# hsinnan75/GSAlign

Hardware: AMD Instinct MI355X
Metric: aligned query Gbp/s (whole node) (higher is better)
Workload: dtype u8; 1 GPU; full-human-sized pair (BASELINE configs[4]): 24 contigs with GRCh38 chromosome lengths, 3.08 Gbp, repeat injection, vs 1; inflight_contexts_per_gpu=8, world_size=1, parallelism=one GPU

## Files before the change

### gsalign_amd/csrc/k_seed.hip

```cpp
#include <cstring>
#include <mutex>
#include <condition_variable>
#include <vector>
#include "gsa_ctx.h"
#include "gsa_fm.h"
#include "gsa_scan.h"

enum { CNT_OCCBLK = 0, CNT_DONE = 1, CNT_HITS = 2, CNT_SEEDS = 3, CNT_DPCELLS = 4, CNT_DPJOBS = 5, CNT_DPMN = 6, CNT_CAND = 8, CNT_OVERFLOW = 9, CNT_OCCBLK_ALL = 10, CNT_HEAVY = 12 };

#ifndef SEED_WG
#define SEED_WG 64
#endif
#ifndef NSUB
#define NSUB 96
#endif
#ifndef ADV_STEPS
#define ADV_STEPS 4
#endif
#ifndef PLOOK
#define PLOOK 3
#endif
#define PATH_WORDS 320
#define QP_WORDS (GSA_CHUNK / 16 + 4)
#define QN_WORDS (GSA_CHUNK / 32 + 4)
// ... 8 lines not shown
{
	const u64 lo = (u64)w0 | ((u64)w1 << 32);
	return sh ? (lo >> sh) | ((u64)w2 << (64 - sh)) : lo;
}
__device__ __forceinline__ u64 q_bits64(const u32 *qp, int p) { const int w = p >> 4; return funnel64(qp[w], qp[w + 1], qp[w + 2], (p & 15) << 1); }
__device__ __forceinline__ u32 q_nbits32(const u32 *qn, int p) { const int w = p >> 5; return (u32)((((u64)qn[w + 1] << 32) | qn[w]) >> (p & 31)); }

__device__ __forceinline__ int text_match32(u32 r0, u32 r1, u32 r2, i64 tp, i64 tend, const u32 *qp, const u32 *qn, int pos, int clen)
{
	int avail = clen - pos;
	if (tend - tp < (i64)avail) avail = (int)(tend - tp);
	if (avail > 32) avail = 32;
	if (avail <= 0) return 0;
	const u64 d = funnel64(r0, r1, r2, (int)(tp & 15) << 1) ^ q_bits64(qp, pos);
	const u64 dm = (d | (d >> 1)) & 0x5555555555555555ull;
	const u32 nm = q_nbits32(qn, pos);
	int n = dm ? (__ffsll((unsigned long long)dm) - 1) >> 1 : 32;
	const int fn = nm ? __ffs((int)nm) - 1 : 32;
	n = n < fn ? n : fn;
	return n < avail ? n : avail;
}

__device__ __forceinline__ u32 pres4_line(u64 qb, int K) { return (u32)((qb >> 6) & ((1ull << (2 * (K - 3))) - 1)); }
__device__ __forceinline__ u32 pres4_bit(u64 qb, int K, int i)
{
	const u32 head = (u32)(qb >> (2 * i)) & ((1u << (2 * (3 - i))) - 1);
	const u32 tail = (u32)(qb >> (2 * K)) & ((1u << (2 * i)) - 1);
	return (u32)i * 64u + (head | (tail << (2 * (3 - i))));
}

template <int TPB>
__device__ __forceinline__ void wg_exscan_hits(const i32 *hits, i32 *base, int n1)
{
	constexpr int V = TPB <= 64 ? 16 : 8;
	__shared__ i32 s_ws[TPB / 64], s_run;
	const int tid = threadIdx.x, lane = tid & 63, wv = tid >> 6;
	if (tid == 0) s_run = 0;
	__syncthreads();
	for (int b0 = 0; b0 < n1; b0 += TPB * V) {
		i32 v[V], tsum = 0;
#pragma unroll
		for (int k = 0; k < V; k++) { const int idx = b0 + tid * V + k; v[k] = idx < n1 ? __hip_atomic_load(&hits[idx], __ATOMIC_RELAXED, __HIP_MEMORY_SCOPE_AGENT) : 0; }
#pragma unroll
		for (int k = 0; k < V; k++) tsum += v[k];
		i32 inc = tsum;
		for (int o = 1; o < 64; o <<= 1) { const i32 t = __shfl_up(inc, o); if (lane >= o) inc += t; }
		if (lane == 63) s_ws[wv] = inc;
		__syncthreads();
		i32 wo = 0, tot = 0;
		for (int w = 0; w < TPB / 64; w++) { const i32 x = s_ws[w]; if (w < wv) wo += x; tot += x; }
		i32 e = s_run + wo + inc - tsum;
#pragma unroll
		for (int k = 0; k < V; k++) { const int idx = b0 + tid * V + k; if (idx < n1) base[idx] = e; e += v[k]; }
		__syncthreads();
		if (tid == 0) s_run += tot;
		__syncthreads();
	}
}

__device__ __forceinline__ void wave_exscan_hits(const i32 *hits, i32 *base, int n1)
{
	constexpr int V = 16;
	const int lane = threadIdx.x & 63;
	i32 run = 0;
	for (int b0 = 0; b0 < n1; b0 += 64 * V) {
		i32 v[V], tsum = 0;
#pragma unroll
		for (int k = 0; k < V; k++) { const int idx = b0 + lane * V + k; v[k] = idx < n1 ? __hip_atomic_load(&hits[idx], __ATOMIC_RELAXED, __HIP_MEMORY_SCOPE_AGENT) : 0; }
#pragma unroll
		for (int k = 0; k < V; k++) tsum += v[k];
		i32 inc = tsum;
		for (int o = 1; o < 64; o <<= 1) { const i32 t = __shfl_up(inc, o); if (lane >= o) inc += t; }
		i32 e = run + inc - tsum;
#pragma unroll
		for (int k = 0; k < V; k++) { const int idx = b0 + lane * V + k; if (idx < n1) base[idx] = e; e += v[k]; }
		run += __shfl(inc, 63);
	}
}

#ifndef SEED_MIN_WAVES
#define SEED_MIN_WAVES 5
#endif
#ifndef LHOP_N
#define LHOP_N 1024
#endif
#define MEMO_WORDS (GSA_CHUNK / 16)
__device__ __forceinline__ int memo_nib(const u32 *memo, int s) { return (int)((memo[s >> 4] >> ((s & 15) << 1)) & 3u); }
__device__ __forceinline__ void memo_one(u32 *memo, int s) { atomicOr(&memo[s >> 4], 1u << ((s & 15) << 1)); }
__device__ __forceinline__ int memo_get(const u32 *memo, const u32 *lhop, int s)
{
	const int v = memo_nib(memo, s);
	if (v < 2) return v;
	if (v == 2) return 5;
	for (u32 h = ((u32)s * 40503u) >> 6;; h++) { const u32 e = lhop[h & (LHOP_N - 1)]; if ((e >> 16) == (u32)s + 1) return (int)(e & 0xffffu); }
}
__device__ __forceinline__ void memo_set(u32 *memo, u32 *lhop, int s, int d, int *abort_flag)
{
	if (d == 1 || d == 5) { atomicOr(&memo[s >> 4], (d == 1 ? 1u : 2u) << ((s & 15) << 1)); return; }
	const u32 e = ((u32)(s + 1) << 16) | (u32)d;
	u32 h = ((u32)s * 40503u) >> 6;
	for (int tries = 0; tries < LHOP_N; tries++, h++) {
		const u32 old = atomicCAS(&lhop[h & (LHOP_N - 1)], 0u, e);
		if (old == 0 || old == e) { atomicOr(&memo[s >> 4], 3u << ((s & 15) << 1)); return; }
	}
	*(volatile int *)abort_flag = 1;
}

__device__ __forceinline__ u32 nt4_quad(u32 w)
{
	const u32 l = w | 0x20202020u;
	const u32 x = (l >> 1) & 0x03030303u;
	u32 code = x ^ ((x >> 1) & 0x01010101u);
	const u32 want = __builtin_amdgcn_perm(0u, 0x74676361u, code);
	const u32 diff = l ^ want;
	const u32 bad = ((diff | ((diff & 0x7f7f7f7fu) + 0x7f7f7f7fu)) >> 7) & 0x01010101u;
	code &= ~(bad * 3u);
	return ((code * 0x01041040u) >> 24) | (((bad * 0x01020408u) >> 24) & 15u) << 8;
}

__device__ __forceinline__ void stage32(const uint8_t *src, int p0, int clen, u32 &w0, u32 &w1, u32 &wn)
{
	u32 d[8];
	if (p0 + 32 <= clen) { const uint4 a = *(const uint4 *)src, b = *(const uint4 *)(src + 16); d[0] = a.x; d[1] = a.y; d[2] = a.z; d[3] = a.w; d[4] = b.x; d[5] = b.y; d[6] = b.z; d[7] = b.w; }
	else {
#pragma unroll
		for (int t = 0; t < 8; t++) { d[t] = 0; for (int k = 0; k < 4; k++) d[t] |= (u32)(p0 + 4 * t + k < clen ? src[4 * t + k] : (uint8_t)'N') << (8 * k); }
	}
	w0 = w1 = wn = 0;
#pragma unroll
	for (int t = 0; t < 8; t++) {
		const u32 r = nt4_quad(d[t]);
		if (t < 4) w0 |= (r & 0xffu) << (8 * t); else w1 |= (r & 0xffu) << (8 * (t - 4));
		wn |= (r >> 8) << (4 * t);
	}
}

template <bool COUNT, int NCH>
struct SeedLds {
	static constexpr int NV = NCH * NSUB;
	u32 s_ncand[NCH], s_queue, s_hits[NCH];
	int changed, s_abort;
	u32 qp[NCH][QP_WORDS], qn[NCH][QN_WORDS];
	u32 memo[NCH][MEMO_WORDS];
	u32 lhop[NCH][LHOP_N];
	uint16_t mblk[COUNT ? GSA_CHUNK : 1];
	u32 bits[NCH][PATH_WORDS];
	uint16_t entry_of[NV], exit_of[NV];
	uint16_t pend_it[SEED_WG];
	uint16_t jmp[2][NV], walked_from[NV];
	u32 rewalked[(NV + 31) / 32], onchain[(NV + 31) / 32], s_npend;
	int s_last;
};
#define SEED_SYNC() do { if (WPW == 1) __syncthreads(); else { __builtin_amdgcn_fence(__ATOMIC_RELEASE, "wavefront"); __builtin_amdgcn_wave_barrier(); __builtin_amdgcn_fence(__ATOMIC_ACQUIRE, "wavefront"); } } while (0)
#define s_ncand sl_.s_ncand
#define s_queue sl_.s_queue
#define s_hits sl_.s_hits
#define changed sl_.changed
#define s_abort sl_.s_abort
#define qp sl_.qp
#define qn sl_.qn
#define memo sl_.memo
#define lhop sl_.lhop
#define mblk sl_.mblk
#define bits sl_.bits
#define entry_of sl_.entry_of
#define exit_of sl_.exit_of
#define pend_it sl_.pend_it
#define jmp sl_.jmp
#define walked_from sl_.walked_from
#define rewalked sl_.rewalked
#define onchain sl_.onchain
#define s_npend sl_.s_npend
#define s_last sl_.s_last
template <bool COUNT, bool E16, int NCH, int WPW>
__device__ __forceinline__ void seed_chunk(const DevIndex &di, const uint8_t *__restrict__ q, i32 qlen, const Params &prm, u64 *cnt,
                                                      i32 *cand_s, i32 *cand_len, u64 *cand_x0, i32 *cand_freq, u32 cand_cap, u32 *cand_cnt, u32 *onpath, i32 *chunk_hits, u64 *hcnt,
                                                      u32 budget, u32 *heavy_list, i32 *chunk_base, const int chunk0, const u32 n_chunks, SeedLds<COUNT, NCH> &sl_)
{
	constexpr int NV = NCH * NSUB;
	static_assert(!COUNT || NCH == 1, "the accounting build walks one chunk per wave");
	const int j = threadIdx.x & 63;
	const int nch = (u32)chunk0 + NCH <= n_chunks ? NCH : (int)(n_chunks - (u32)chunk0);
	i64 c0[NCH]; int clen[NCH], S[NCH], nitems[NCH]; size_t cbase[NCH];
#pragma unroll
	for (int ch = 0; ch < NCH; ch++) {
		c0[ch] = (i64)(chunk0 + ch) * GSA_CHUNK;
		clen[ch] = ch < nch ? (int)((i64)qlen - c0[ch] < GSA_CHUNK ? (i64)qlen - c0[ch] : GSA_CHUNK) : 0;
		S[ch] = (clen[ch] + NSUB - 1) / NSUB; if (S[ch] < 1) S[ch] = 1;
		nitems[ch] = (clen[ch] + S[ch] - 1) / S[ch];
		cbase[ch] = (size_t)(chunk0 + ch) * cand_cap;
	}
	const int nitems_all = NCH == 1 ? nitems[0] : nitems[0] + nitems[NCH - 1];
#define CH_SEL(ARR, CH) (NCH == 1 ? ARR[0] : ((CH) ? ARR[NCH - 1] : ARR[0]))
#pragma unroll
	for (int ch = 0; ch < NCH; ch++) {
		for (int g = j; g < QN_WORDS; g += SEED_WG) {
			u32 w0 = 0, w1 = 0, wn = 0;
			const int p0 = g << 5;
			if (p0 < clen[ch]) stage32(q + c0[ch] + p0, p0, clen[ch], w0, w1, wn);
			if (2 * g < QP_WORDS) qp[ch][2 * g] = w0;
			if (2 * g + 1 < QP_WORDS) qp[ch][2 * g + 1] = w1;
			qn[ch][g] = wn;
		}
		for (int p = j; p < MEMO_WORDS; p += SEED_WG) memo[ch][p] = 0;
		for (int p = j; p < LHOP_N; p += SEED_WG) lhop[ch][p] = 0;
		for (int p = j; p < PATH_WORDS; p += SEED_WG) bits[ch][p] = 0;
		for (int it = j; it < nitems[ch]; it += SEED_WG) entry_of[ch * NSUB + it] = (uint16_t)(it * S[ch]);
		if (j == 0) { s_ncand[ch] = 0; s_hits[ch] = 0; }
	}
	if (j == 0) { s_queue = 0; s_npend = 0; s_abort = 0; }
	if (j < (NV + 31) / 32) rewalked[j] = 0;
	u32 all_blocks = 0, rounds = 0, iters = 0;
#ifdef SEED_STATS
	u32 st_it = 0, st_fm_any = 0, st_fm_only = 0, st_act = 0, st_fm = 0;
#endif
	unsigned long long t_begin = wall_clock64(), t_round0 = 0, t_resolve = 0;
	u32 dirty = 0;
	int fb_item = 0;
	SEED_SYNC();
	for (;;) {
		int item = -1, s = 0, bend = 0, pos = 0, mode = M_ADV; u32 kid = 0, pid = 0, pext = 0;
		int lclen = 0;
		const u32 *qp_l = qp[0], *qn_l = qn[0]; u32 *memo_l = memo[0], *lhop_l = lhop[0];
		FmIntv ik = {0, 0, 0}; u32 blk = 0; i64 tp = 0;
		i64 mp[4] = {0, 0, 0, 0}; u32 malive = 0;
		bool need_item = true;
		while (!__all(mode == M_DONE)) {
			iters++;
			if (!COUNT && budget && iters > budget) *(volatile int *)&s_abort = 1;
			if (*(volatile int *)&s_abort) break;
#ifdef SEED_STATS
			{ const u64 bf = __ballot(mode == M_FM), ba = __ballot(mode != M_DONE);
			  st_it++; st_fm_any += bf != 0; st_fm_only += bf != 0 && bf == ba; st_act += __popcll(ba); st_fm += __popcll(bf); }
#endif
			u64 kk = 0, ll = 0; bool kn = true, ln = true;
			if (mode == M_FM) {
				const u64 k = ik.x1 - 1, l = ik.x1 - 1 + ik.x2;
				kn = (k == (u64)-1); ln = (l == (u64)-1);
				kk = kn ? 0 : k - (k >= di.primary); ll = ln ? 0 : l - (l >= di.primary);
			}
#ifdef SEED_SKIP_IDLE
#define ANY_IN(M) __any(mode == (M))
#else
#define ANY_IN(M) true
#endif
			FmBlock bk = {{0, 0, 0, 0}, {0, 0, 0, 0}, 0, 0, 0, 0}, bl = bk;
			if (ANY_IN(M_FM)) { bk = fm_load(di, kk >> 6); bl = fm_load(di, ll >> 6); }
			struct __attribute__((packed, aligned(4))) W5 { u32 a, b, c, d, e; };
			W5 w5 = {0, 0, 0, 0, 0};
			if (ANY_IN(M_TEXT)) w5 = *(const W5 *)(di.ref2 + (mode == M_TEXT ? (tp >> 4) : ((mode == M_MTEXT && (malive & 1u)) ? (mp[0] >> 4) : 0)));
			const u32 r0 = w5.a, r1 = w5.b, r2 = w5.c, r3 = w5.d, r4 = w5.e;
			ulonglong2 e0 = {0, 0}, e1 = {0, 0};
			if (!ANY_IN(M_KMER)) {}
			else if (E16) {
				const uint4 e = ((const uint4 *)(di.kmer ? di.kmer : (const u64 *)di.bwt))[mode == M_KMER ? kid : 0];
				e0.x = e.x; e0.y = e.y; e1.x = e.z; e1.y = e.w;
			} else {
				const ulonglong2 *pe = (const ulonglong2 *)((di.kmer ? di.kmer : (const u64 *)di.bwt) + (mode == M_KMER ? ((size_t)kid << 2) : 0));
				e0 = pe[0]; e1 = pe[1];
			}
			uint4 pl0 = {~0u, ~0u, ~0u, ~0u}, pl1 = {~0u, ~0u, ~0u, ~0u};
			if (di.pres && ANY_IN(M_KMER)) { const uint4 *pp = (const uint4 *)di.pres + 2 * (size_t)(mode == M_KMER ? pid : 0); pl0 = pp[0]; pl1 = pp[1]; }
#define PRES4_TEST(I) ((((((pext >> (2 * (I))) & 32u) ? ((I) == 0 ? pl0.y : (I) == 1 ? pl0.w : (I) == 2 ? pl1.y : pl1.w) : ((I) == 0 ? pl0.x : (I) == 1 ? pl0.z : (I) == 2 ? pl1.x : pl1.z)) >> ((pext >> (2 * (I))) & 31u)) & 1u) != 0)
			u64 sav = 0;
			if (ANY_IN(M_LOC)) sav = fm_locate(di, (mode == M_LOC || mode == M_MLOC) ? ik.x0 : 1);
#undef ANY_IN
			u64 sav1 = 0, sav2 = 0, sav3 = 0; W5 w5b = {0, 0, 0, 0, 0}, w5c = w5b, w5d = w5b;
			if (!COUNT && SEED_MULTI > 1) {
				if (__any(mode == M_MLOC)) {
					const int nr = mode == M_MLOC ? (int)ik.x2 : 0;
					sav1 = fm_locate(di, nr > 1 ? ik.x0 + 1 : 1); sav2 = fm_locate(di, nr > 2 ? ik.x0 + 2 : 1); sav3 = fm_locate(di, nr > 3 ? ik.x0 + 3 : 1);
				}
				if (__any(mode == M_MTEXT)) {
					const bool mt = mode == M_MTEXT;
					w5b = *(const W5 *)(di.ref2 + ((mt && (malive & 2u)) ? (mp[1] >> 4) : 0));
					w5c = *(const W5 *)(di.ref2 + ((mt && (malive & 4u)) ? (mp[2] >> 4) : 0));
					w5d = *(const W5 *)(di.ref2 + ((mt && (malive & 8u)) ? (mp[3] >> 4) : 0));
				}
			}
			bool ended = false;
			if (mode == M_KMER) {
				if (!PRES4_TEST(0)) {
					memo_one(memo_l, s); s += 1; mode = M_ADV;
					const int L = prm.MinSeedLength < 32 ? prm.MinSeedLength : 32;
#pragma unroll
					for (int k2 = 0; k2 < PLOOK; k2++) {
						if (s >= bend || memo_nib(memo_l, s)) break;
						const u32 nb = q_nbits32(qn_l, s);
						if (s + prm.MinSeedLength > lclen || (nb & (L == 32 ? ~0u : (1u << L) - 1)) != 0) break;
						if (k2 == 0 ? PRES4_TEST(1) : k2 == 1 ? PRES4_TEST(2) : PRES4_TEST(3)) break;
						memo_one(memo_l, s); s += 1;
					}
				} else {
					const bool hit = e1.x != 0;
					if (hit) { ik.x0 = e0.x; ik.x1 = e0.y; ik.x2 = e1.x; pos = s + di.kmer_k; }
					else ik = fm_init(di, q_code(qp_l, s));
					mode = M_FM;
					if (hit && ik.x2 == 1) { tp = (i64)(e1.y - 1) + di.kmer_k; mode = M_TEXT; }
					else if (!COUNT && SEED_MULTI > 1 && hit && ik.x2 <= SEED_MULTI) mode = M_MLOC;
				}
			} else if (mode == M_LOC) {
				tp = (i64)sav + (pos - s); mode = M_TEXT;
			} else if (!COUNT && SEED_MULTI > 1 && mode == M_MLOC) {
				mp[0] = (i64)sav + (pos - s); mp[1] = (i64)sav1 + (pos - s); mp[2] = (i64)sav2 + (pos - s); mp[3] = (i64)sav3 + (pos - s);
				malive = (1u << (int)ik.x2) - 1u; mode = M_MTEXT;
			} else if (!COUNT && SEED_MULTI > 1 && mode == M_MTEXT) {
				int g0 = -1, g1 = -1, g2 = -1, g3 = -1;
#define MT_ROW(G, W, P) { int got = text_match32(W.a, W.b, W.c, P, (i64)di.seq_len, qp_l, qn_l, pos, lclen); if (got == 32) got += text_match32(W.c, W.d, W.e, P + 32, (i64)di.seq_len, qp_l, qn_l, pos + 32, lclen); G = got; }
				if (malive & 1u) MT_ROW(g0, w5, mp[0])
				if (malive & 2u) MT_ROW(g1, w5b, mp[1])
				if (malive & 4u) MT_ROW(g2, w5c, mp[2])
				if (malive & 8u) MT_ROW(g3, w5d, mp[3])
#undef MT_ROW
				int m = g0 > g1 ? g0 : g1; m = m > g2 ? m : g2; m = m > g3 ? m : g3;
				const u32 na = (g0 == m ? 1u : 0u) | (g1 == m ? 2u : 0u) | (g2 == m ? 4u : 0u) | (g3 == m ? 8u : 0u);
				pos += m; mp[0] += m; mp[1] += m; mp[2] += m; mp[3] += m;
				if (m < 64 || __popc(na) == 1) {
					const int first = __ffs((int)na) - 1;
					ik.x0 += (u64)first; ik.x2 = (u64)__popc(na);
					if (m == 64) { tp = first == 0 ? mp[0] : first == 1 ? mp[1] : first == 2 ? mp[2] : mp[3]; mode = M_TEXT; }
					else ended = true;
				} else malive = na;
				if (mode == M_MTEXT && !ended && malive != na) malive = na;
			} else if (mode == M_TEXT) {
				int got = text_match32(r0, r1, r2, tp, (i64)di.seq_len, qp_l, qn_l, pos, lclen);
				if (got == 32) got += text_match32(r2, r3, r4, tp + 32, (i64)di.seq_len, qp_l, qn_l, pos + 32, lclen);
				pos += got; tp += got;
				ended = got < 64;
			} else if (mode == M_FM) {
				const bool can = pos < lclen && !q_isn(qn_l, pos < lclen ? pos : 0);
				const bool ok = can && fm_extend_loaded(di, ik, q_code(qp_l, pos < lclen ? pos : 0), bk, bl, kk, ll, kn, ln, blk);
				ended = !ok;
				if (ok) { pos++; if (!COUNT && ik.x2 == 1) mode = M_LOC; else if (!COUNT && SEED_MULTI > 1 && ik.x2 <= SEED_MULTI) mode = M_MLOC; }
			}
			if (ended) {
				const int len = pos - s;
				int d = 1;
				if (len >= prm.MinSeedLength && ik.x2 <= GSA_MAX_SEED_FREQ) {
					const int ch = NCH == 1 ? 0 : (item >= NSUB ? NCH - 1 : 0);
					const u32 slot = atomicAdd(&s_ncand[ch], 1u);
					const size_t cb = CH_SEL(cbase, ch);
					if (slot < cand_cap) { cand_s[cb + slot] = (i32)(CH_SEL(c0, ch) + s); cand_len[cb + slot] = len; cand_x0[cb + slot] = ik.x0; cand_freq[cb + slot] = (i32)ik.x2; }
					else cnt[CNT_OVERFLOW] = 1;
					d = prm.bSensitive ? 5 : len + 1;
				}
				memo_set(memo_l, lhop_l, s, d, &s_abort); if (COUNT) mblk[s] = (uint16_t)blk;
				all_blocks += blk;
				s += d; mode = M_ADV;
			}
			for (int step = 0; step < ADV_STEPS && mode == M_ADV; step++) {
				if (need_item) {
					if (rounds == 0) {
						const u32 it_ = atomicAdd(&s_queue, 1u);
						if (NCH == 1) item = it_ < (u32)nitems[0] ? (int)it_ : -1;
						else {
							const u32 both = 2u * (u32)(nitems[0] < nitems[NCH - 1] ? nitems[0] : nitems[NCH - 1]);
							if (it_ < both) item = (int)(it_ >> 1) + ((it_ & 1u) ? NSUB : 0);
							else if (it_ < (u32)nitems_all) { const int r = (int)(it_ - both) + (int)(both >> 1); item = nitems[0] > nitems[NCH - 1] ? r : NSUB + r; }
							else item = -1;
						}
					}
					else if (dirty) { dirty = 0; item = fb_item; }
					else item = -1;
					need_item = false;
					if (item < 0) { mode = M_DONE; break; }
					const int ch = NCH == 1 ? 0 : (item >= NSUB ? NCH - 1 : 0), li = item - ch * NSUB;
					lclen = CH_SEL(clen, ch); qp_l = qp[ch]; qn_l = qn[ch]; memo_l = memo[ch]; lhop_l = lhop[ch];
					const int S_l = CH_SEL(S, ch);
					s = entry_of[item]; bend = (li + 1) * S_l < lclen ? (li + 1) * S_l : lclen;
				}
				if (s >= bend) { exit_of[item] = (uint16_t)s; need_item = true; continue; }
				const int m_ = memo_get(memo_l, lhop_l, s);
				if (m_) { s += m_; continue; }
				const u32 nb = q_nbits32(qn_l, s);
				const int L = prm.MinSeedLength < 32 ? prm.MinSeedLength : 32;
				if (nb & 1u) { memo_one(memo_l, s); if (COUNT) mblk[s] = 0; s += 1; }
				else if (!COUNT && (s + prm.MinSeedLength > lclen || (nb & (L == 32 ? ~0u : (1u << L) - 1)) != 0)) { memo_one(memo_l, s); s += 1; }
				else {
					pos = s + 1; blk = 0; mode = M_FM;
#ifdef SEED_EAGER_INIT
					ik = fm_init(di, q_code(qp_l, s));
#endif
					if (COUNT || !(di.kmer_k > 1 && s + di.kmer_k <= lclen && (nb & ((1u << di.kmer_k) - 1)) == 0)) ik = fm_init(di, q_code(qp_l, s));
					else {
						const u64 qb = q_bits64(qp_l, s);
						kid = (u32)(qb & ((1ull << (2 * di.kmer_k)) - 1)); mode = M_KMER;
						pid = di.pres_k ? pres4_line(qb, di.pres_k) : 0;
						pext = di.pres_k ? (((u32)qb & 63u) | (((u32)(qb >> (2 * di.pres_k)) & 63u) << 6)) : 0;
					}
				}
			}
		}
#undef PRES4_TEST
		rounds++;
		SEED_SYNC();
		if (s_abort) break;
		if (rounds == 1) t_round0 = wall_clock64() - t_begin;
		const unsigned long long t_r0 = wall_clock64();
#define V_LIVE(V) ((V) < NSUB ? (V) < nitems[0] : (NCH > 1 && (V) - NSUB < nitems[NCH - 1]))
		for (int v = j; v < NV; v += SEED_WG) if (V_LIVE(v)) {
			const int ch = v >= NSUB ? NCH - 1 : 0;
			const int X = exit_of[v]; jmp[0][v] = (uint16_t)(X >= CH_SEL(clen, ch) ? 0xffff : ch * NSUB + X / CH_SEL(S, ch));
		}
		if (j < (NV + 31) / 32) onchain[j] = 0;
		if (j == 0) s_npend = 0;
		SEED_SYNC();
		if (j == 0) { onchain[0] = 1u; if (NCH > 1 && nitems[NCH - 1] > 0) atomicOr(&onchain[NSUB >> 5], 1u << (NSUB & 31)); }
		SEED_SYNC();
		int cur = 0;
		const int nmax = NCH == 1 ? nitems[0] : (nitems[0] > nitems[NCH - 1] ? nitems[0] : nitems[NCH - 1]);
		for (int span = 1; span < nmax; span <<= 1) {
			for (int v = j; v < NV; v += SEED_WG) if (V_LIVE(v)) {
				const int t = jmp[cur][v];
				if (t != 0xffff) {
					if ((onchain[v >> 5] >> (v & 31)) & 1u) atomicOr(&onchain[t >> 5], 1u << (t & 31));
					jmp[cur ^ 1][v] = jmp[cur][t];
				} else jmp[cur ^ 1][v] = 0xffff;
			}
			SEED_SYNC();
			cur ^= 1;
		}
		for (int v = j; v < NV; v += SEED_WG) if (V_LIVE(v)) { const int ch = v >= NSUB ? NCH - 1 : 0; entry_of[v] = (uint16_t)((v - ch * NSUB) ? CH_SEL(clen, ch) : 0); }
		SEED_SYNC();
		for (int v = j; v < NV; v += SEED_WG) if (V_LIVE(v))
			if ((onchain[v >> 5] >> (v & 31)) & 1u) { const int ch = v >= NSUB ? NCH - 1 : 0; const int X = exit_of[v]; if (X < CH_SEL(clen, ch)) entry_of[ch * NSUB + X / CH_SEL(S, ch)] = (uint16_t)X; }
		SEED_SYNC();
		for (int v = j; v < NV; v += SEED_WG) if (V_LIVE(v)) {
			if (!((onchain[v >> 5] >> (v & 31)) & 1u)) continue;
			const int ch = v >= NSUB ? NCH - 1 : 0;
			const int e = entry_of[v];
			const bool known = ((rewalked[v >> 5] >> (v & 31)) & 1u) ? e == walked_from[v] : memo_nib(memo[ch], e) != 0;
			if (!known) {
				const u32 idx = atomicAdd(&s_npend, 1u);
				if (idx < SEED_WG) { pend_it[idx] = (uint16_t)v; walked_from[v] = (uint16_t)e; atomicOr(&rewalked[v >> 5], 1u << (v & 31)); }
			}
		}
		SEED_SYNC();
		if (j == 0) { if (s_npend > SEED_WG) s_npend = SEED_WG; changed = s_npend > 0 ? 1 : 0; }
		SEED_SYNC();
		t_resolve += wall_clock64() - t_r0;
		const int again = changed;
		if (again && j < (int)s_npend) { fb_item = pend_it[j]; dirty = 1; }
		SEED_SYNC();
		if (!again) break;
	}
	const bool heavy = s_abort != 0;
	if (heavy) {
		if (j == 0) for (int ch = 0; ch < nch; ch++) {
			const u32 hslot = (u32)atomicAdd((unsigned long long *)&cnt[CNT_HEAVY], 1ull);
			heavy_list[hslot] = (u32)(chunk0 + ch);
			s_ncand[ch] = 0; cand_cnt[chunk0 + ch] = 0; lb_pub(&chunk_hits[chunk0 + ch], 0); if (chunk0 + ch == 0) lb_pub(&chunk_hits[n_chunks], 0);
		}
		SEED_SYNC();
	}
	u32 alg_blocks = 0;
	if (!heavy) for (int v = j; v < NV; v += SEED_WG) if (V_LIVE(v)) {
		const int ch = v >= NSUB ? NCH - 1 : 0, li = v - ch * NSUB;
		const int bend = (li + 1) * CH_SEL(S, ch) < CH_SEL(clen, ch) ? (li + 1) * CH_SEL(S, ch) : CH_SEL(clen, ch);
		for (int s = entry_of[v]; s < bend;) { atomicOr(&bits[ch][s >> 5], 1u << (s & 31)); if (COUNT) alg_blocks += mblk[s]; s += memo_get(memo[ch], lhop[ch], s); }
	}
#undef V_LIVE
	for (int o = 32; o; o >>= 1) { alg_blocks += __shfl_down(alg_blocks, o); all_blocks += __shfl_down(all_blocks, o); }
	if ((j & 63) == 0) {
		if (alg_blocks) atomicAdd((unsigned long long *)&cnt[CNT_OCCBLK], (unsigned long long)alg_blocks);
		if (all_blocks) atomicAdd((unsigned long long *)&cnt[CNT_OCCBLK_ALL], (unsigned long long)all_blocks);
#ifndef SEED_STATS
		atomicMax((unsigned long long *)&cnt[13], (unsigned long long)iters);
#endif
	}
#ifdef SEED_STATS
	if ((j & 63) == 0) { atomicAdd((unsigned long long *)&cnt[11], (unsigned long long)st_it); atomicAdd((unsigned long long *)&cnt[13], (unsigned long long)st_fm_any); atomicAdd((unsigned long long *)&cnt[14], (unsigned long long)st_fm_only);
	                     atomicAdd((unsigned long long *)&cnt[15], (unsigned long long)st_act); atomicAdd((unsigned long long *)&cnt[7], (unsigned long long)st_fm); }
	if (false)
#endif
	if (j == 0) { atomicMax((unsigned long long *)&cnt[11], (unsigned long long)rounds); atomicMax((unsigned long long *)&cnt[14], t_round0); atomicMax((unsigned long long *)&cnt[15], t_resolve); atomicMax((unsigned long long *)&cnt[7], wall_clock64() - t_begin); }
	SEED_SYNC();
	if (!heavy) {
#pragma unroll
		for (int ch = 0; ch < NCH; ch++) if (ch < nch) {
			for (int p = j; p < PATH_WORDS; p += SEED_WG) onpath[(size_t)(chunk0 + ch) * PATH_WORDS + p] = bits[ch][p];
			const u32 nc = s_ncand[ch] < cand_cap ? s_ncand[ch] : cand_cap;
			u32 h = 0;
			for (u32 i = j; i < nc; i += SEED_WG) { const i32 p = cand_s[cbase[ch] + i] - (i32)c0[ch]; if ((bits[ch][p >> 5] >> (p & 31)) & 1u) h += (u32)cand_freq[cbase[ch] + i]; }
			for (int o = 32; o; o >>= 1) h += __shfl_down(h, o);
			if ((j & 63) == 0 && h) atomicAdd(&s_hits[ch], h);
		}
		SEED_SYNC();
		if (j == 0) for (int ch = 0; ch < nch; ch++) {
			const u32 nc = s_ncand[ch] < cand_cap ? s_ncand[ch] : cand_cap;
			cand_cnt[chunk0 + ch] = nc; lb_pub(&chunk_hits[chunk0 + ch], (i32)s_hits[ch]); if (chunk0 + ch == 0) lb_pub(&chunk_hits[n_chunks], 0); atomicMax((unsigned long long *)&cnt[CNT_CAND], (unsigned long long)s_ncand[ch]);
			if (s_hits[ch]) atomicAdd((unsigned long long *)&cnt[CNT_HITS], (unsigned long long)s_hits[ch]);
		}
	}
#undef CH_SEL
	asm volatile("s_waitcnt vmcnt(0)" ::: "memory");
	SEED_SYNC();
	if (j == 0) {
		__builtin_amdgcn_fence(__ATOMIC_RELEASE, "workgroup");
		s_last = atomicAdd((unsigned long long *)&cnt[CNT_DONE], (unsigned long long)nch) == (unsigned long long)n_chunks - (unsigned long long)nch ? 1 : 0;
	}
	SEED_SYNC();
	if (s_last && j < 16) {
		hcnt[j] = j == CNT_DONE ? 0 : __hip_atomic_load(&cnt[j], __ATOMIC_RELAXED, __HIP_MEMORY_SCOPE_AGENT);
		cnt[j] = 0;
	}
	if (s_last) { if (WPW == 1) wg_exscan_hits<SEED_WG>(chunk_hits, chunk_base, (int)n_chunks + 1); else wave_exscan_hits(chunk_hits, chunk_base, (int)n_chunks + 1); }
}
#undef s_ncand
#undef s_queue
#undef s_hits
#undef changed
#undef s_abort
#undef qp
#undef qn
#undef memo
#undef lhop
#undef mblk
#undef bits
#undef entry_of
#undef exit_of
#undef pend_it
#undef jmp
#undef walked_from
#undef rewalked
#undef onchain
#undef s_npend
#undef s_last
#undef SEED_SYNC


#define SEED_TICKET 16
#ifndef SEED_PERSIST
#define SEED_PERSIST 12
#endif
#ifndef SEED_NCH
#define SEED_NCH 1
#endif
#ifndef SEED_WPW
#define SEED_WPW 8
#endif
#ifndef SEED_WGS_PER_CU
#define SEED_WGS_PER_CU 1
#endif
#define SEED_WG_LDS_MIN ((160 * 1024) / (SEED_WGS_PER_CU + 1) + 2048)
#define SEED_LB_WAVES(COUNT_) ((COUNT_) ? 1 : SEED_MIN_WAVES)
template <bool COUNT, bool E16>
__global__ void __launch_bounds__(SEED_WG * (COUNT ? 1 : SEED_WPW), SEED_LB_WAVES(COUNT)) k_seed_wg(DevIndex di, const uint8_t *__restrict__ q, i32 qlen, Params prm, u64 *cnt,
                                                      i32 *cand_s, i32 *cand_len, u64 *cand_x0, i32 *cand_freq, u32 cand_cap, u32 *cand_cnt, u32 *onpath, i32 *chunk_hits, u64 *hcnt,
                                                      u32 budget, u32 *heavy_list, i32 *chunk_base, u64 tk_base, u32 n_chunks)
{
	constexpr int NCH = COUNT ? 1 : SEED_NCH;
	constexpr int WPW = COUNT ? 1 : SEED_WPW;
	typedef SeedLds<COUNT, NCH> Lds;
	extern __shared__ __attribute__((aligned(16))) unsigned char seed_dyn_lds[];
	Lds *lds = (Lds *)seed_dyn_lds;
	Lds &L = lds[WPW == 1 ? 0 : (threadIdx.x >> 6)];
	for (;;) {
		u32 unit = 0;
		if ((threadIdx.x & 63) == 0) unit = (u32)(atomicAdd((unsigned long long *)&cnt[SEED_TICKET], 1ull) - tk_base);
		unit = (u32)__builtin_amdgcn_readfirstlane((int)unit);
		if ((u64)unit * NCH >= n_chunks) return;
		seed_chunk<COUNT, E16, NCH, WPW>(di, q, qlen, prm, cnt, cand_s, cand_len, cand_x0, cand_freq, cand_cap, cand_cnt, onpath, chunk_hits, hcnt, budget, heavy_list, chunk_base, (int)(unit * NCH), n_chunks, L);
	}
}


#define DENSE_TPB 256
#define DENSE_WGS(SPAN) ((GSA_CHUNK + (SPAN) - 1) / (SPAN))
template <bool E16, int DENSE_SPAN>
__global__ void __launch_bounds__(DENSE_TPB) k_dense_search(DevIndex di, const uint8_t *__restrict__ q, i32 qlen, Params prm, const u32 *__restrict__ chunk_list,
                                                              u32 *dn_lf, u64 *dn_x0, u64 *cnt)
{
	__shared__ u32 qp[QP_WORDS], qn[QN_WORDS];
	const u32 slot = blockIdx.x / DENSE_WGS(DENSE_SPAN), part = blockIdx.x % DENSE_WGS(DENSE_SPAN);
	const u32 chunk = chunk_list ? chunk_list[slot] : slot;
	const int j = threadIdx.x;
	const i64 c0 = (i64)chunk * GSA_CHUNK;
	const int clen = (int)((i64)qlen - c0 < GSA_CHUNK ? (i64)qlen - c0 : GSA_CHUNK);
	const int span0 = (int)part * DENSE_SPAN, span1 = span0 + DENSE_SPAN < clen ? span0 + DENSE_SPAN : clen;
	if (span0 >= clen) return;
	for (int g = (span0 >> 5) + j; g < QN_WORDS; g += DENSE_TPB) {
		u32 w0 = 0, w1 = 0, wn = 0;
		const int p0 = g << 5;
		if (p0 < clen) {
			stage32(q + c0 + p0, p0, clen, w0, w1, wn);
		}
		if (2 * g < QP_WORDS) qp[2 * g] = w0;
		if (2 * g + 1 < QP_WORDS) qp[2 * g + 1] = w1;
		qn[g] = wn;
	}
	__syncthreads();
	u32 *lf = dn_lf + (size_t)slot * GSA_CHUNK; u64 *x0o = dn_x0 + (size_t)slot * GSA_CHUNK;
	int nextp = span0 + j;
	int s = 0, pos = 0, mode = M_ADV; u32 kid = 0, pid = 0, pext = 0, blk = 0, all_blocks = 0;
	FmIntv ik = {0, 0, 0}; i64 tp = 0;
	const int L = prm.MinSeedLength < 32 ? prm.MinSeedLength : 32;
	while (!__all(mode == M_DONE)) {
		u64 kk = 0, ll = 0; bool kn = true, ln = true;
		if (mode == M_FM) {
			const u64 k = ik.x1 - 1, l = ik.x1 - 1 + ik.x2;
			kn = (k == (u64)-1); ln = (l == (u64)-1);
			kk = kn ? 0 : k - (k >= di.primary); ll = ln ? 0 : l - (l >= di.primary);
		}
		const FmBlock bk = fm_load(di, kk >> 6), bl = fm_load(di, ll >> 6);
		struct __attribute__((packed, aligned(4))) W5 { u32 a, b, c, d, e; };
		const W5 w5 = *(const W5 *)(di.ref2 + (mode == M_TEXT ? (tp >> 4) : 0));
		ulonglong2 e0 = {0, 0}, e1 = {0, 0};
		if (E16) {
			const uint4 e = ((const uint4 *)(di.kmer ? di.kmer : (const u64 *)di.bwt))[mode == M_KMER ? kid : 0];
			e0.x = e.x; e0.y = e.y; e1.x = e.z; e1.y = e.w;
		} else {
			const ulonglong2 *pe = (const ulonglong2 *)((di.kmer ? di.kmer : (const u64 *)di.bwt) + (mode == M_KMER ? ((size_t)kid << 2) : 0));
			e0 = pe[0]; e1 = pe[1];
		}
		ulonglong2 l0 = {0, 0}, l1 = {0, 0};
		if (di.kmer_lo) {
			if (E16) { const uint4 e = ((const uint4 *)di.kmer_lo)[mode == M_KLO ? kid : 0]; l0.x = e.x; l0.y = e.y; l1.x = e.z; l1.y = e.w; }
			else { const ulonglong2 *pe = (const ulonglong2 *)(di.kmer_lo + (mode == M_KLO ? ((size_t)kid << 2) : 0)); l0 = pe[0]; l1 = pe[1]; }
		}
		const u32 pw = di.pres ? di.pres[mode == M_KMER ? pid : 0] : ~0u;
		const u64 sav = fm_locate(di, mode == M_LOC ? ik.x0 : 1);
		bool ended = false;
		if (mode == M_KMER) {
			if (!((pw >> pext) & 1u)) { ended = true; pos = s; ik.x2 = 0; }
			else {
				const bool hit = e1.x != 0;
				if (hit) { ik.x0 = e0.x; ik.x1 = e0.y; ik.x2 = e1.x; pos = s + di.kmer_k; }
// ... 864 lines not shown
	return GSA_OK;
}

static std::mutex g_seed_mu; static std::condition_variable g_seed_cv; static int g_seed_busy[64];
struct SeedGate {
	int dev, slots; bool held;
	SeedGate(int d, int n) : dev(d & 63), slots(n), held(false) { if (slots > 0) { std::unique_lock<std::mutex> lk(g_seed_mu); g_seed_cv.wait(lk, [&] { return g_seed_busy[dev] < slots; }); g_seed_busy[dev]++; held = true; } }
	void release() { if (held) { { std::lock_guard<std::mutex> lk(g_seed_mu); g_seed_busy[dev]--; } g_seed_cv.notify_all(); held = false; } }
	~SeedGate() { release(); }
};

int stage1_seed(gsa_ctx *c)
{
#ifdef GSA_EXPERIMENTS
	static const int seed_cus = [] { const char *e = getenv("GSA_SEED_CUS"); return e ? atoi(e) : 0; }();
#else
	const int seed_cus = 0;
#endif
	if (seed_cus > 0 && !c->stream_seed) {
		hipDeviceProp_t pr; GSA_CHECK(c, hipGetDeviceProperties(&pr, c->device));
		const int ncu = pr.multiProcessorCount;
		std::vector<uint32_t> mask((size_t)(ncu + 31) / 32, 0u);
		for (int i = 0; i < ncu; i++) if ((long long)(i + 1) * seed_cus / ncu != (long long)i * seed_cus / ncu) mask[(size_t)i >> 5] |= 1u << (i & 31);
		GSA_CHECK(c, hipExtStreamCreateWithCUMask(&c->stream_seed, (uint32_t)mask.size(), mask.data()));
		GSA_CHECK(c, hipEventCreateWithFlags(&c->ev_seed_fork, hipEventDisableTiming));
	}
	hipStream_t st = c->stream;
	if (c->stream_seed) {
		GSA_CHECK(c, hipEventRecord(c->ev_seed_fork, c->stream)); GSA_CHECK(c, hipStreamWaitEvent(c->stream_seed, c->ev_seed_fork, 0));
		st = c->stream_seed;
	}
	const bool split = c->split;
	const i64 all_chunks = ((i64)c->qlen + GSA_CHUNK - 1) / GSA_CHUNK;
	const i64 cb = split ? c->rng_beg : 0, ce = split ? (c->rng_end < all_chunks ? c->rng_end : all_chunks) : all_chunks;
	const i32 s_off = (i32)(cb * GSA_CHUNK);
	const i32 qlen_full = c->qlen;
	const i32 qlen = ce > cb ? (i32)(((i64)ce * GSA_CHUNK < (i64)qlen_full ? (i64)ce * GSA_CHUNK : (i64)qlen_full) - s_off) : 0;
	const uint8_t *d_q = c->q_dev + s_off;
	c->n_seeds = 0; c->n_groups = 0;
	if (qlen <= 0) return split ? prepare_pd_bitmap(c, 0) : GSA_OK;
	const i64 n_chunks = ((i64)qlen + GSA_CHUNK - 1) / GSA_CHUNK;
	size_t ccap = c->cand_cap_per_chunk;
	if (!dev_ensure<u32>(c, c->d_onpath, (size_t)n_chunks * PATH_WORDS) || !dev_ensure<i32>(c, c->d_chunk_hits, (size_t)n_chunks + 1) || !dev_ensure<i32>(c, c->d_chunk_base, (size_t)n_chunks + 1)) return GSA_ERR_NOMEM;
	i64 n_hits = 0;
	u64 *cnt = c->d_cnt.as<u64>();
	const int seed_mode = c->opt.seed_mode;
	const bool sweep_all = !c->prm.bSensitive && !c->count_blocks && (seed_mode == 0 || (seed_mode == 1 && c->seed_sweep_next));
	const bool dense_all = (c->prm.bSensitive || sweep_all) && !c->count_blocks;
	const u32 budget = c->count_blocks ? 0u : c->seed_budget;
	if (dense_all && ccap < GSA_CHUNK / 5 + 64) { ccap = GSA_CHUNK / 5 + 64; c->cand_cap_per_chunk = ccap; }
	u64 occ_all = 0;
#ifdef GSA_EXPERIMENTS
	static const int seed_slots = [] { const char *e = getenv("GSA_SEED_SLOTS"); return e ? atoi(e) : 0; }();
#else
	const int seed_slots = 0;
#endif
	SeedGate gate(c->device, (c->profiling || c->count_blocks) ? 0 : seed_slots);
	u64 contig_maxcand = 0;
	for (int attempt = 0;; attempt++) {
		if (attempt == 8) return gsa_fail(c, GSA_ERR_LIMIT, "seed buffers keep overflowing");
		const size_t ctot = ccap * (size_t)n_chunks;
		if (!dev_ensure<i32>(c, c->d_cand_s, ctot) || !dev_ensure<i32>(c, c->d_cand_len, ctot) || !dev_ensure<u64>(c, c->d_cand_x0, ctot) || !dev_ensure<i32>(c, c->d_cand_freq, ctot) || !dev_ensure<u32>(c, c->d_cand_cnt, (size_t)n_chunks)) return GSA_ERR_NOMEM;
		if (!dense_all && !dev_ensure<u32>(c, c->d_heavy, (size_t)n_chunks)) return GSA_ERR_NOMEM;
		if (c->profiling || c->prof_seed) hipEventRecord(c->ev[0], st);
		u64 hits = 0, maxcand = 0, n_heavy = dense_all ? (u64)n_chunks : 0;
		occ_all = 0;
		if (!dense_all) {
#define GSA_SEED_ARGS c->di, d_q, qlen, c->prm, cnt, c->d_cand_s.as<i32>(), c->d_cand_len.as<i32>(), c->d_cand_x0.as<u64>(), c->d_cand_freq.as<i32>(), (u32)ccap, \
			c->d_cand_cnt.as<u32>(), c->d_onpath.as<u32>(), c->d_chunk_hits.as<i32>(), c->h_cnt, budget, c->d_heavy.as<u32>(), c->d_chunk_base.as<i32>()
			const i64 n_units = c->count_blocks ? n_chunks : (n_chunks + SEED_NCH - 1) / SEED_NCH;
			const int wpw = c->count_blocks ? 1 : SEED_WPW;
			unsigned grid = (unsigned)((n_units + wpw - 1) / wpw);
			if (!c->count_blocks) {
				if (c->n_cus <= 0) { hipDeviceProp_t pr; GSA_CHECK(c, hipGetDeviceProperties(&pr, c->device)); c->n_cus = pr.multiProcessorCount; }
				const i64 cap = (i64)c->n_cus * (SEED_WPW > 1 ? SEED_WGS_PER_CU : SEED_PERSIST);
				if (cap < (i64)grid) grid = (unsigned)cap;
			}
			const u64 tk_base = c->seed_ticket; c->seed_ticket += (u64)n_units + (u64)grid * (u64)wpw;
			const size_t dl_count = sizeof(SeedLds<true, 1>);
			size_t dl = sizeof(SeedLds<false, SEED_NCH>) * SEED_WPW; if (SEED_WPW > 1 && dl < SEED_WG_LDS_MIN) dl = SEED_WG_LDS_MIN;
			if (c->count_blocks) hipLaunchKernelGGL((k_seed_wg<true, false>), dim3(grid), dim3(SEED_WG), dl_count, st, GSA_SEED_ARGS, tk_base, (u32)n_chunks);
			else if (c->di.kmer_e16) hipLaunchKernelGGL((k_seed_wg<false, true>), dim3(grid), dim3(SEED_WG * SEED_WPW), dl, st, GSA_SEED_ARGS, tk_base, (u32)n_chunks);
			else hipLaunchKernelGGL((k_seed_wg<false, false>), dim3(grid), dim3(SEED_WG * SEED_WPW), dl, st, GSA_SEED_ARGS, tk_base, (u32)n_chunks);
#undef GSA_SEED_ARGS
			if (c->profiling || c->prof_seed) hipEventRecord(c->ev[1], st);
			GSA_CHECK(c, hipEventRecord(c->ev[21], st));
			GSA_CHECK(c, hipEventSynchronize(c->ev[21]));
			hits = c->h_cnt[CNT_HITS]; maxcand = c->h_cnt[CNT_CAND]; n_heavy = c->h_cnt[CNT_HEAVY]; occ_all = c->h_cnt[CNT_OCCBLK_ALL];
			c->dbg[0] = c->h_cnt[11]; c->dbg[1] = n_heavy; c->dbg[2] = c->h_cnt[13]; c->dbg[3] = c->h_cnt[14]; c->dbg[4] = c->h_cnt[15]; c->dbg[5] = c->h_cnt[7];
			c->counters[0] = c->h_cnt[CNT_OCCBLK];
			if (seed_mode == 1) {
				c->seed_sweep_next = n_heavy * 5 > (u64)n_chunks * 2;
				c->seed_sweep_period = (c->seed_sweep_next && c->seed_sweep_probe) ? (c->seed_sweep_period < 64 ? c->seed_sweep_period * 2 : 64) : 8;
				c->seed_sweep_probe = false;
			}
		}
		if (n_heavy > 0) {
			const size_t nd = (size_t)n_heavy * GSA_CHUNK;
			if (!dev_ensure<u32>(c, c->dn_lf, nd) || !dev_ensure<u64>(c, c->dn_x0, nd)) return GSA_ERR_NOMEM;
			const u32 *list = dense_all ? (const u32 *)nullptr : c->d_heavy.as<u32>();
#define GSA_DENSE_ARGS(SPAN) dim3((unsigned)(n_heavy * DENSE_WGS(SPAN))), dim3(DENSE_TPB), 0, st, c->di, d_q, qlen, c->prm, list, c->dn_lf.as<u32>(), c->dn_x0.as<u64>(), cnt
#ifdef GSA_EXPERIMENTS
			static const u64 sweep_min = [] { const char *e = getenv("GSA_SWEEP_MIN"); return e ? (u64)atoll(e) : 1024ull; }();
#else
			const u64 sweep_min = 1024;
#endif
			const bool use_sweep = seed_mode != 2 && ((seed_mode == 0 && dense_all) || n_heavy >= sweep_min);
			if (sweep_all && seed_mode == 1 && ++c->seed_sweep_run >= c->seed_sweep_period) { c->seed_sweep_next = false; c->seed_sweep_probe = true; c->seed_sweep_run = 0; }
			if (use_sweep) {
#ifdef GSA_EXPERIMENTS
				static const int seg_env = [] { const char *e = getenv("GSA_SWEEP_SEG"); return e ? atoi(e) : 0; }();
#else
				const int seg_env = 0;
#endif
				const int shape_env = c->opt.sweep_shape;
				const bool small = shape_env >= 0 ? shape_env == 1 : n_heavy < 4096;
				const int seg = seg_env > 0 ? seg_env : (small ? 40 : 160);
#define GSA_SWEEP_ARGS(NCH_, TPB_) dim3((unsigned)((n_heavy + (NCH_) - 1) / (NCH_))), dim3(TPB_), 0, st, c->di, d_q, qlen, c->prm, list, (u32)n_heavy, c->dn_lf.as<u32>(), c->dn_x0.as<u64>(), cnt, seg
				if (small) { if (c->di.kmer_e16) hipLaunchKernelGGL((k_dense_sweep<true, 1, 256>), GSA_SWEEP_ARGS(1, 256)); else hipLaunchKernelGGL((k_dense_sweep<false, 1, 256>), GSA_SWEEP_ARGS(1, 256)); }
				else { if (c->di.kmer_e16) hipLaunchKernelGGL((k_dense_sweep<true, SWEEP_NCH, SWEEP_TPB>), GSA_SWEEP_ARGS(SWEEP_NCH, SWEEP_TPB)); else hipLaunchKernelGGL((k_dense_sweep<false, SWEEP_NCH, SWEEP_TPB>), GSA_SWEEP_ARGS(SWEEP_NCH, SWEEP_TPB)); }
#undef GSA_SWEEP_ARGS
			}
			else if (dense_all) { if (c->di.kmer_e16) hipLaunchKernelGGL((k_dense_search<true, 512>), GSA_DENSE_ARGS(512)); else hipLaunchKernelGGL((k_dense_search<false, 512>), GSA_DENSE_ARGS(512)); }
			else { if (c->di.kmer_e16) hipLaunchKernelGGL((k_dense_search<true, 256>), GSA_DENSE_ARGS(256)); else hipLaunchKernelGGL((k_dense_search<false, 256>), GSA_DENSE_ARGS(256)); }
#undef GSA_DENSE_ARGS
			hipLaunchKernelGGL(k_dense_resolve, dim3((unsigned)n_heavy), dim3(256), 0, st, list, (u32)n_chunks, qlen, (int)c->prm.bSensitive, c->dn_lf.as<u32>(), c->dn_x0.as<u64>(), cnt,
			                   c->d_cand_s.as<i32>(), c->d_cand_len.as<i32>(), c->d_cand_x0.as<u64>(), c->d_cand_freq.as<i32>(), (u32)ccap, c->d_cand_cnt.as<u32>(), c->d_onpath.as<u32>(),
			                   c->d_chunk_hits.as<i32>(), c->h_cnt, c->d_chunk_base.as<i32>());
			GSA_CHECK(c, hipGetLastError());
			if (c->profiling || c->prof_seed) hipEventRecord(c->ev[1], st);
			GSA_CHECK(c, hipEventRecord(c->ev[21], st));
			GSA_CHECK(c, hipEventSynchronize(c->ev[21]));
			hits += c->h_cnt[CNT_HITS]; if (c->h_cnt[CNT_CAND] > maxcand) maxcand = c->h_cnt[CNT_CAND]; occ_all += c->h_cnt[CNT_OCCBLK_ALL];
			if (dense_all) { c->dbg[0] = 0; c->dbg[1] = n_heavy; c->dbg[2] = c->dbg[3] = c->dbg[4] = c->dbg[5] = 0; c->counters[0] = 0; }
		}
		if (hits >= (1ull << 31) - 2) return gsa_fail(c, GSA_ERR_LIMIT, "more than 2^31 seeds in one contig");
		if (maxcand > ccap) { ccap = (size_t)maxcand + 256; c->cand_cap_per_chunk = ccap; continue; }
		n_hits = (i64)hits; contig_maxcand = maxcand;
		break;
	}
	gate.release();
	st = c->stream;
	const size_t hcap = (size_t)n_hits + 64;
	if (int rcp = prepare_pd_bitmap(c, n_hits, n_chunks)) return rcp;
	if (n_hits > 0) {
		if (!dev_ensure<u64>(c, c->d_key_a, hcap) || !dev_ensure<u32>(c, c->d_val_a, hcap)) return GSA_ERR_NOMEM;
		const size_t sel_cand = contig_maxcand < ccap ? (((size_t)contig_maxcand + 64) & ~(size_t)63) : ccap;
		hipLaunchKernelGGL(k_seed_select, dim3((unsigned)n_chunks), dim3(256), 2 * (sel_cand + 2) * sizeof(u32), st, c->di, (u32)ccap, c->d_cand_cnt.as<u32>(), c->d_cand_s.as<i32>(), c->d_cand_len.as<i32>(),
		                   c->d_cand_x0.as<u64>(), c->d_cand_freq.as<i32>(), c->d_onpath.as<u32>(), c->d_chunk_base.as<i32>(), c->bnd, s_off, c->qbits, c->d_key_a.as<u64>(), c->d_val_a.as<u32>(), c->pd_path ? c->d_pdbm.as<u32>() : (u32 *)nullptr, c->d_pdcb.as<u32>(), (u32)sel_cand, (c->pd_path && c->pd_bytes) ? c->d_pdby.as<uint8_t>() : (uint8_t *)nullptr);
		if (c->pd_path && c->pd_bytes) {
			const i64 tiles = (c->pd_words + 1023) >> 10;
			hipLaunchKernelGGL(k_pd_pack, dim3((unsigned)(tiles < 4096 ? tiles : 4096)), dim3(256), 0, st, c->d_pdby.as<uint8_t>(), c->pd_words, c->d_pdbm.as<u32>(), c->d_pdcb.as<u32>());
		}
	}
	if (c->profiling) hipEventRecord(c->ev[2], st);
	u64 lf_steps = 0;
	if (c->count_blocks && n_hits > 0) {
		unsigned long long *d_lf = (unsigned long long *)(c->d_mail.as<i32>() + M_LFSTEPS);
		GSA_CHECK(c, hipMemsetAsync(d_lf, 0, 8, st));
		hipLaunchKernelGGL(k_count_lf, dim3((unsigned)n_chunks), dim3(256), 0, st, c->di, (u32)ccap, c->d_cand_cnt.as<u32>(), c->d_cand_s.as<i32>(), c->d_cand_x0.as<u64>(),
		                   c->d_cand_freq.as<i32>(), c->d_onpath.as<u32>(), d_lf);
		GSA_CHECK(c, hipMemcpyAsync(&c->h_cnt[CNT_DONE], d_lf, 8, hipMemcpyDeviceToHost, st));
		GSA_CHECK(c, hipStreamSynchronize(st));
		lf_steps = c->h_cnt[CNT_DONE];
	}
	c->counters[1] = lf_steps; c->counters[2] = (u64)n_hits; c->counters[3] = (u64)n_hits; c->counters[7] = occ_all;
// ... 114 lines not shown
```

Baseline: 33.31 Gbp/s.

## Shrink per-chunk seed LDS state by aliasing path bits onto query mask and halving hop table

Shrinks the seed kernel's per-chunk LDS state so more chunk states fit per workgroup or CU. It halves the long-hop memo hash table (except in the counting build) and stores the path bitmap in the same LDS as the query N-mask, which is no longer needed once the walk finishes. The bitmap is now cleared after the walk, with extra syncs around it. The smaller hash table fills sooner, so more chunks may set the abort flag and fall back to the heavy path, and the aliasing relies on qn being dead by that point.

```diff
diff --git a/gsalign_amd/csrc/k_seed.hip b/gsalign_amd/csrc/k_seed.hip
--- a/gsalign_amd/csrc/k_seed.hip
+++ b/gsalign_amd/csrc/k_seed.hip
@@ -114,25 +114,27 @@
 #define SEED_MIN_WAVES 5
 #endif
 #ifndef LHOP_N
-#define LHOP_N 1024
+#define LHOP_N 512
 #endif
 #define MEMO_WORDS (GSA_CHUNK / 16)
 __device__ __forceinline__ int memo_nib(const u32 *memo, int s) { return (int)((memo[s >> 4] >> ((s & 15) << 1)) & 3u); }
 __device__ __forceinline__ void memo_one(u32 *memo, int s) { atomicOr(&memo[s >> 4], 1u << ((s & 15) << 1)); }
+template <int LN>
 __device__ __forceinline__ int memo_get(const u32 *memo, const u32 *lhop, int s)
 {
 	const int v = memo_nib(memo, s);
 	if (v < 2) return v;
 	if (v == 2) return 5;
-	for (u32 h = ((u32)s * 40503u) >> 6;; h++) { const u32 e = lhop[h & (LHOP_N - 1)]; if ((e >> 16) == (u32)s + 1) return (int)(e & 0xffffu); }
-}
+	for (u32 h = ((u32)s * 40503u) >> 6;; h++) { const u32 e = lhop[h & (LN - 1)]; if ((e >> 16) == (u32)s + 1) return (int)(e & 0xffffu); }
+}
+template <int LN>
 __device__ __forceinline__ void memo_set(u32 *memo, u32 *lhop, int s, int d, int *abort_flag)
 {
 	if (d == 1 || d == 5) { atomicOr(&memo[s >> 4], (d == 1 ? 1u : 2u) << ((s & 15) << 1)); return; }
 	const u32 e = ((u32)(s + 1) << 16) | (u32)d;
 	u32 h = ((u32)s * 40503u) >> 6;
-	for (int tries = 0; tries < LHOP_N; tries++, h++) {
-		const u32 old = atomicCAS(&lhop[h & (LHOP_N - 1)], 0u, e);
+	for (int tries = 0; tries < LN; tries++, h++) {
+		const u32 old = atomicCAS(&lhop[h & (LN - 1)], 0u, e);
 		if (old == 0 || old == e) { atomicOr(&memo[s >> 4], 3u << ((s & 15) << 1)); return; }
 	}
 	*(volatile int *)abort_flag = 1;
@@ -172,17 +174,19 @@
 	static constexpr int NV = NCH * NSUB;
 	u32 s_ncand[NCH], s_queue, s_hits[NCH];
 	int changed, s_abort;
-	u32 qp[NCH][QP_WORDS], qn[NCH][QN_WORDS];
+	u32 qp[NCH][QP_WORDS];
+	union { u32 qn[NCH][QN_WORDS]; u32 bits[NCH][PATH_WORDS]; };
 	u32 memo[NCH][MEMO_WORDS];
-	u32 lhop[NCH][LHOP_N];
+	static constexpr int LN = COUNT ? 1024 : LHOP_N;
+	u32 lhop[NCH][LN];
 	uint16_t mblk[COUNT ? GSA_CHUNK : 1];
-	u32 bits[NCH][PATH_WORDS];
 	uint16_t entry_of[NV], exit_of[NV];
 	uint16_t pend_it[SEED_WG];
 	uint16_t jmp[2][NV], walked_from[NV];
 	u32 rewalked[(NV + 31) / 32], onchain[(NV + 31) / 32], s_npend;
 	int s_last;
 };
+static_assert(sizeof(SeedLds<false, 1>) <= 10240, "ten chunk states per workgroup: SeedLds<false, 1> must stay at 10 KB or less");
 #define SEED_SYNC() do { if (WPW == 1) __syncthreads(); else { __builtin_amdgcn_fence(__ATOMIC_RELEASE, "wavefront"); __builtin_amdgcn_wave_barrier(); __builtin_amdgcn_fence(__ATOMIC_ACQUIRE, "wavefront"); } } while (0)
 #define s_ncand sl_.s_ncand
 #define s_queue sl_.s_queue
@@ -210,6 +214,7 @@
                                                       u32 budget, u32 *heavy_list, i32 *chunk_base, const int chunk0, const u32 n_chunks, SeedLds<COUNT, NCH> &sl_)
 {
 	constexpr int NV = NCH * NSUB;
+	constexpr int LN = SeedLds<COUNT, NCH>::LN;
 	static_assert(!COUNT || NCH == 1, "the accounting build walks one chunk per wave");
 	const int j = threadIdx.x & 63;
 	const int nch = (u32)chunk0 + NCH <= n_chunks ? NCH : (int)(n_chunks - (u32)chunk0);
@@ -235,8 +240,7 @@
 			qn[ch][g] = wn;
 		}
 		for (int p = j; p < MEMO_WORDS; p += SEED_WG) memo[ch][p] = 0;
-		for (int p = j; p < LHOP_N; p += SEED_WG) lhop[ch][p] = 0;
-		for (int p = j; p < PATH_WORDS; p += SEED_WG) bits[ch][p] = 0;
+		for (int p = j; p < LN; p += SEED_WG) lhop[ch][p] = 0;
 		for (int it = j; it < nitems[ch]; it += SEED_WG) entry_of[ch * NSUB + it] = (uint16_t)(it * S[ch]);
 		if (j == 0) { s_ncand[ch] = 0; s_hits[ch] = 0; }
 	}
@@ -376,7 +380,7 @@
 					else cnt[CNT_OVERFLOW] = 1;
 					d = prm.bSensitive ? 5 : len + 1;
 				}
-				memo_set(memo_l, lhop_l, s, d, &s_abort); if (COUNT) mblk[s] = (uint16_t)blk;
+				memo_set<LN>(memo_l, lhop_l, s, d, &s_abort); if (COUNT) mblk[s] = (uint16_t)blk;
 				all_blocks += blk;
 				s += d; mode = M_ADV;
 			}
@@ -402,7 +406,7 @@
 					s = entry_of[item]; bend = (li + 1) * S_l < lclen ? (li + 1) * S_l : lclen;
 				}
 				if (s >= bend) { exit_of[item] = (uint16_t)s; need_item = true; continue; }
-				const int m_ = memo_get(memo_l, lhop_l, s);
+				const int m_ = memo_get<LN>(memo_l, lhop_l, s);
 				if (m_) { s += m_; continue; }
 				const u32 nb = q_nbits32(qn_l, s);
 				const int L = prm.MinSeedLength < 32 ? prm.MinSeedLength : 32;
@@ -486,10 +490,16 @@
 		SEED_SYNC();
 	}
 	u32 alg_blocks = 0;
+	SEED_SYNC();
+	if (!heavy) {
+#pragma unroll
+		for (int ch = 0; ch < NCH; ch++) for (int p = j; p < PATH_WORDS; p += SEED_WG) bits[ch][p] = 0;
+	}
+	SEED_SYNC();
 	if (!heavy) for (int v = j; v < NV; v += SEED_WG) if (V_LIVE(v)) {
 		const int ch = v >= NSUB ? NCH - 1 : 0, li = v - ch * NSUB;
 		const int bend = (li + 1) * CH_SEL(S, ch) < CH_SEL(clen, ch) ? (li + 1) * CH_SEL(S, ch) : CH_SEL(clen, ch);
-		for (int s = entry_of[v]; s < bend;) { atomicOr(&bits[ch][s >> 5], 1u << (s & 31)); if (COUNT) alg_blocks += mblk[s]; s += memo_get(memo[ch], lhop[ch], s); }
+		for (int s = entry_of[v]; s < bend;) { atomicOr(&bits[ch][s >> 5], 1u << (s & 31)); if (COUNT) alg_blocks += mblk[s]; s += memo_get<LN>(memo[ch], lhop[ch], s); }
 	}
 #undef V_LIVE
 	for (int o = 32; o; o >>= 1) { alg_blocks += __shfl_down(alg_blocks, o); all_blocks += __shfl_down(all_blocks, o); }
@@ -575,6 +585,7 @@
 #define SEED_WGS_PER_CU 1
 #endif
 #define SEED_WG_LDS_MIN ((160 * 1024) / (SEED_WGS_PER_CU + 1) + 2048)
+static_assert(SEED_WG == 64 || SEED_WPW == 1, "the independent waves of a fat workgroup own one chunk each: a chunk's lanes are one wave");
 #define SEED_LB_WAVES(COUNT_) ((COUNT_) ? 1 : SEED_MIN_WAVES)
 template <bool COUNT, bool E16>
 __global__ void __launch_bounds__(SEED_WG * (COUNT ? 1 : SEED_WPW), SEED_LB_WAVES(COUNT)) k_seed_wg(DevIndex di, const uint8_t *__restrict__ q, i32 qlen, Params prm, u64 *cnt,
@@ -1605,6 +1616,7 @@
 			if (c->count_blocks) hipLaunchKernelGGL((k_seed_wg<true, false>), dim3(grid), dim3(SEED_WG), dl_count, st, GSA_SEED_ARGS, tk_base, (u32)n_chunks);
 			else if (c->di.kmer_e16) hipLaunchKernelGGL((k_seed_wg<false, true>), dim3(grid), dim3(SEED_WG * SEED_WPW), dl, st, GSA_SEED_ARGS, tk_base, (u32)n_chunks);
 			else hipLaunchKernelGGL((k_seed_wg<false, false>), dim3(grid), dim3(SEED_WG * SEED_WPW), dl, st, GSA_SEED_ARGS, tk_base, (u32)n_chunks);
+			GSA_CHECK(c, hipGetLastError());
 #undef GSA_SEED_ARGS
 			if (c->profiling || c->prof_seed) hipEventRecord(c->ev[1], st);
 			GSA_CHECK(c, hipEventRecord(c->ev[21], st));
```

Result: slower. 32.81 Gbp/s (-1.5%).
